# Deltares/xugrid

Hardware: AMD Instinct MI355X
Metric: target cells regridded/s (OverlapRegridder 1M->1M tri, weights + mean apply) (higher is better)
Workload: dtype f64; 1 GPU; BASELINE config 2: ~1M-triangle jittered-lattice Delaunay source -> ~1M-triangle target (seed 1, rotated 30 deg, scaled 0.7), OverlapRegridder area-weighted mean, K=1; target_faces=999660, candidate_pairs=6677422, nnz=4052965, parallelism=1 GPU

## Files before the change

xugrid_amd/csrc/xr_clip_tri.h:

```cpp
#pragma once

#include "xr_geom.h"

namespace xr {

static constexpr double TRI_AREA_OVERFLOW = -1.0;
static constexpr int TRI_MAXV = 6;
static constexpr int TRI_LUT = 64;

template <int MAXV>
__device__ __forceinline__ void poly_lut_init(uint2 *lut) {
    constexpr int N_LUT = 1 << MAXV;
    const int i = threadIdx.x;
    if (i >= N_LUT) return;
    uint32_t pos[8] = {MAXV, MAXV, MAXV, MAXV, MAXV, MAXV, MAXV, MAXV};
    if (i >= 8) {
        const int n = 31 - __clz(i);
        const uint32_t F = (uint32_t)i - (1u << n);
        int before = 0, n_t = 0;
        for (int j = 0; j < n; j++) {
            const bool fj = (F >> j) & 1u, fp = (F >> ((j + n - 1) % n)) & 1u;
            if (fj != fp) {
                if (n_t < 2) pos[5 + n_t] = (uint32_t)before;
                n_t++;
// ... 36 lines not shown
            const bool cross = live && (b_inside != a_inside);
            P2 pt{0.0, 0.0};
            bool have_pt = false;
            if (cross) {
                const double wx = r.x - a.x, wy = r.y - a.y;
                const double nw = N.x * wx + N.y * wy;
                const double nv = N.x * V.x + N.y * V.y;
                if (nv != 0) {
                    const double tt = nw / nv;
                    pt.x = a.x + tt * V.x;
                    pt.y = a.y + tt * V.y;
                    have_pt = true;
                }
            }
            const bool quirk = cross && !b_inside && !have_pt;
            if (cross && have_pt) {
                col[(n_output < MAXV ? n_output : MAXV) * STRIDE] = make_double2(pt.x, pt.y);
                n_output++;
            }
            b_inside = b_inside || quirk;
            if (live && b_inside) {
                col[(n_output < MAXV ? n_output : MAXV) * STRIDE] = make_double2(b.x, b.y);
                n_output++;
            }
            if (live) {
                a = b;
                a_inside = b_inside;
            }
        }
    }
    if (n_output > MAXV) {
        overflow = true;
        alive = false;
    } else if (n_output < 3) {
        alive = false;
    }
    n = n_output;
}

template <int MAXV, int NIN, int STRIDE, bool LAST = false>
__device__ __forceinline__ void poly_stage(int &n, P2 &r, const P2 s, bool &alive, bool &dirty, bool &overflow,
                                           double2 *col, const uint2 *lut) {
    const P2 U{s.x - r.x, s.y - r.y};
    const bool work = alive && !(U.x == 0 && U.y == 0);
    P2 v[MAXV];
#pragma unroll
    for (int j = 0; j < MAXV; j++) {
        if (j < NIN) {
            const double2 q = col[j * STRIDE];
            v[j] = P2{q.x, q.y};
        } else {
            v[j] = P2{0.0, 0.0};
        }
    }
    uint32_t F = 0;
#pragma unroll
    for (int j = 0; j < NIN; j++) F |= (U.x * (v[j].y - r.y) > U.y * (v[j].x - r.x)) ? (1u << j) : 0u;
    const uint32_t nmask = (1u << n) - 1u;
    F &= nmask;
    const uint32_t Tm = (F ^ ((F << 1) | (F >> ((n - 1) & 31)))) & nmask;
    const int n_tr = __popc(Tm);
    bool irregular = work && (dirty || n > NIN || (n_tr != 0 && n_tr != 2));
    const bool two = work && !irregular && n_tr == 2;
    if (two) {
        const int j1 = __ffs(Tm) - 1, j2 = 31 - __clz(Tm);
        const int p1 = j1 == 0 ? n - 1 : j1 - 1, p2 = j2 - 1;
        const double2 a1 = col[p1 * STRIDE], b1 = col[j1 * STRIDE], a2 = col[p2 * STRIDE], b2 = col[j2 * STRIDE];
        const uint2 e = lut[F + (1u << n)];
        const P2 N{-U.y, U.x};
        const P2 V1{b1.x - a1.x, b1.y - a1.y}, V2{b2.x - a2.x, b2.y - a2.y};
        const double nw1 = N.x * (r.x - a1.x) + N.y * (r.y - a1.y), nv1 = N.x * V1.x + N.y * V1.y;
        const double nw2 = N.x * (r.x - a2.x) + N.y * (r.y - a2.y), nv2 = N.x * V2.x + N.y * V2.y;
        const double tt1 = nw1 / nv1, tt2 = nw2 / nv2;
        const P2 pt1{a1.x + tt1 * V1.x, a1.y + tt1 * V1.y}, pt2{a2.x + tt2 * V2.x, a2.y + tt2 * V2.y};
        irregular = nv1 == 0 || nv2 == 0;
        if (!irregular) {
            if (!LAST && (pt1.x == a1.x || pt1.x == b1.x || pt2.x == a2.x || pt2.x == b2.x || pt1.x == pt2.x))
                dirty = p2_eq(pt1, a1) || p2_eq(pt1, b1) || p2_eq(pt2, a2) || p2_eq(pt2, b2) || p2_eq(pt1, pt2);
            *tri_slot<STRIDE>(col, e.x & 0xffu) = make_double2(v[0].x, v[0].y);
            *tri_slot<STRIDE>(col, (e.x >> 8) & 0xffu) = make_double2(v[1].x, v[1].y);
            *tri_slot<STRIDE>(col, (e.x >> 16) & 0xffu) = make_double2(v[2].x, v[2].y);
            if (NIN > 3) *tri_slot<STRIDE>(col, e.x >> 24) = make_double2(v[3].x, v[3].y);
            if (NIN > 4) *tri_slot<STRIDE>(col, e.y & 0xffu) = make_double2(v[4].x, v[4].y);
            if (NIN > 5) *tri_slot<STRIDE>(col, e.y >> 24) = make_double2(v[5].x, v[5].y);
            *tri_slot<STRIDE>(col, (e.y >> 8) & 0xffu) = make_double2(pt1.x, pt1.y);
            *tri_slot<STRIDE>(col, (e.y >> 16) & 0xffu) = make_double2(pt2.x, pt2.y);
            n = __popc(F) + 2;
        }
    } else if (work && !irregular && !(F & 1u)) {
        alive = false;
    }
    if (irregular) {
        if (n > NIN) {
#pragma unroll
            for (int j = NIN; j < MAXV; j++) {
                if (j < n) {
                    const double2 q = col[j * STRIDE];
                    v[j] = P2{q.x, q.y};
                }
            }
        }
        poly_stage_generic<MAXV, STRIDE>(v, n, r, U, alive, overflow, col);
        dirty = true;
    }
    if (work) r = s;
}

template <int MAXV, int N0, int STRIDE = 1>
__device__ __forceinline__ double poly_clip_area(const P2 (&tv)[N0], int n0, const P2 (&sv)[3], double2 *col, const uint2 *lut,
                                                 bool active) {
    int n = n0;
    bool alive = active, overflow = false;
    bool dirty = false;
#pragma unroll
    for (int j = 0; j < N0; j++)
        if (j < n0) dirty = dirty || p2_eq(tv[j], tv[j + 1 < n0 ? j + 1 : 0]);
    if (N0 > 3 && n0 > 3) dirty = dirty || p2_eq(tv[0], tv[2]) || p2_eq(tv[1], tv[3 < N0 ? 3 : 0]);
    if (active) {
#pragma unroll
        for (int j = 0; j < N0; j++)
            if (j < n0) col[j * STRIDE] = make_double2(tv[j].x, tv[j].y);
    }
    P2 r = sv[2];
    poly_stage<MAXV, N0, STRIDE>(n, r, sv[0], alive, dirty, overflow, col, lut);
    poly_stage<MAXV, N0 + 1, STRIDE>(n, r, sv[1], alive, dirty, overflow, col, lut);
    poly_stage<MAXV, N0 + 2, STRIDE, true>(n, r, sv[2], alive, dirty, overflow, col, lut);
    if (overflow) return TRI_AREA_OVERFLOW;
    double area = 0.0;
    if (alive) {
        const double2 q0 = col[0], q1 = col[STRIDE];
        const P2 a0{q0.x, q0.y};
        double ux = q1.x - a0.x, uy = q1.y - a0.y;
#pragma unroll
        for (int i = 2; i < MAXV; i++) {
            if (i < n) {
                const double2 q = col[i * STRIDE];
                const double vx = a0.x - q.x, vy = a0.y - q.y;
                area += fabs(ux * vy - uy * vx);
                ux = vx;
                uy = vy;
            }
        }
        area = 0.5 * area;
    }
    return area;
}

template <int STRIDE = 1>
__device__ __forceinline__ double tri_clip_area(const P2 (&tv)[3], const P2 (&sv)[3], double2 *col, const uint2 *lut,
                                                bool active) {
    return poly_clip_area<TRI_MAXV, 3, STRIDE>(tv, 3, sv, col, lut, active);
}

static constexpr int QUAD_MAXV = 7;
static constexpr int QUAD_LUT = 1 << QUAD_MAXV;

}
```

xugrid_amd/csrc/xr_overlap.hip:

```cpp
#include "xr_objects.h"
#include "xr_clip_tri.h"

namespace xr {

static constexpr int BIG_VISITS = 160;

__device__ __forceinline__ bool rec_hit(float4 b, float qx0, float qx1, float qy0, float qy1) {
    return box_gap(b, qx0, qx1, qy0, qy1) < 0.0f;
}

static constexpr int SLOTS = 16;
static constexpr int QCUR_STRIDE = 32;
static constexpr int TILE_RUN = 16;

__device__ __forceinline__ int64_t xcd_block(int64_t n_blocks, bool remap) {
    if (!remap) return blockIdx.x;
    const int64_t per_xcd = (n_blocks + 7) >> 3;
    return (int64_t)(blockIdx.x & 7) * per_xcd + (blockIdx.x >> 3);
}

static constexpr int WALK_PAD = 8;
static constexpr int BIGREC_MAX = 1024;
static constexpr int BIGREC_BLOCK = 64;

// ... 285 lines not shown
        if (slot_face && threadIdx.x == 0)
            slot_face[nb <= BIG_RANK_MAX ? sh_rankw[0] + sh_rankw[1] + sh_rankw[2] + sh_rankw[3] : bi] = t;
        if (threadIdx.x < np) sh_poly[threadIdx.x] = reinterpret_cast<const double2 *>(q_fxy)[face_vertex_base(q_off, t, q_m) + threadIdx.x];
        if (threadIdx.x == 0) sh_cursor = 0;
        __syncthreads();
        const double2 *poly = sh_poly;
        const double4 bb = reinterpret_cast<const double4 *>(q_bbox)[t];
        const float qx0 = f32_below(bb.x - g.x0), qx1 = f32_above(bb.y - g.x0);
        const float qy0 = f32_below(bb.z - g.y0), qy1 = f32_above(bb.w - g.y0);
        for (int pass = FUSED ? 0 : 1; pass < 2; pass++) {
        const bool STAGE = pass == 0;
        if (!STAGE) {
            if (FUSED) {
                __syncthreads();
                const int n = sh_cursor;
                __syncthreads();
                if (threadIdx.x == 0) {
                    const int base = atomicAdd(queue_cursor, n);
                    cand_count[t] = n;
                    cand_off[t] = base;
                    const bool fits = (int64_t)base + n <= capacity && base >= 0;
                    if (!fits) pending_list[atomicAdd(n_pending, 1)] = t;
                    sh_out0 = fits ? base : -1;
                    sh_cursor = 0;
                }
                __syncthreads();
                const int out = sh_out0;
                if (out < 0) break;
                if (n <= big_stage) {
                    for (int i = threadIdx.x; i < n; i += 256) {
                        cand_tgt[out + i] = t;
                        cand_src[out + i] = sh_stage[i];
                    }
                    break;
                }
            } else {
                if (threadIdx.x == 0) sh_out0 = cand_off[t];
                __syncthreads();
            }
            if (sh_out0 < 0) break;
        }
        const int out0 = STAGE ? 0 : sh_out0;
        for (int l = 0; l < g.n_levels; l++) {
            const double h = level_h(g, l), inv_h = level_inv_h(g, l);
            const double eps = 1e-6 * h;
            const int nx = g.nx[l], ny = g.ny[l], base = g.base[l];
            const int cy0 = cell_coord(bb.z - h, g.y0, inv_h, ny), cy1 = cell_coord(bb.w, g.y0, inv_h, ny);
            int batch_id = 0;
            for (int cyb = cy0; cyb <= cy1; cyb += 64, batch_id++) {
                if (((batch_id + l) & 3) != wv) continue;
                const int cy = cyb + lane;
                int r0 = 0, r1 = 0;
                float rx0 = qx0, rx1 = qx1;
                if (cy <= cy1) {
                    const double ya = g.y0 + (double)cy * h - eps, yb = g.y0 + (double)(cy + 2) * h + eps;
                    double xlo = INFINITY, xhi = -INFINITY;
                    double2 p = poly[np - 1];
                    for (int k = 0; k < np; k++) {
                        const double2 q = poly[k];
                        const double ylo = fmin(p.y, q.y), yhi = fmax(p.y, q.y);
                        if (yhi >= ya && ylo <= yb) {
                            double xa = p.x, xb = q.x;
                            if (yhi > ylo) {
                                const double inv = 1.0 / (q.y - p.y);
                                double t0 = (ya - p.y) * inv, t1 = (yb - p.y) * inv;
                                if (t0 > t1) { const double tmp = t0; t0 = t1; t1 = tmp; }
                                t0 = fmax(t0, 0.0);
                                t1 = fmin(t1, 1.0);
                                xa = p.x + t0 * (q.x - p.x);
                                xb = p.x + t1 * (q.x - p.x);
                            }
                            xlo = fmin(xlo, fmin(xa, xb));
                            xhi = fmax(xhi, fmax(xa, xb));
                        }
                        p = q;
                    }
                    if (xhi >= xlo) {
                        xlo = fmax(xlo - eps, bb.x);
                        xhi = fmin(xhi + eps, bb.y);
                        const int cx0 = cell_coord(xlo - h, g.x0, inv_h, nx), cx1 = cell_coord(xhi, g.x0, inv_h, nx);
                        r0 = cell_start[base + cy * nx + cx0];
                        r1 = cell_start[base + cy * nx + cx1 + 1];
                        rx0 = fmaxf(qx0, f32_below(xlo - g.x0));
                        rx1 = fminf(qx1, f32_above(xhi - g.x0));
                    }
                }
                const int len = r1 - r0;
                unsigned long long long_mask = __ballot(len > LONG_RUN);
                while (long_mask) {
                    const int src_lane = __ffsll((long long)long_mask) - 1;
                    long_mask &= long_mask - 1;
                    const int R0 = __shfl(r0, src_lane, 64), R1 = __shfl(r1, src_lane, 64);
                    const float X0 = __shfl(rx0, src_lane, 64), X1 = __shfl(rx1, src_lane, 64);
                    for (int rb = R0; rb < R1; rb += 64) {
                        const int r = rb + lane;
                        const bool hit = r < R1 && rec_hit(rbb[r], X0, X1, qy0, qy1);
                        const unsigned long long mask = __ballot(hit);
                        const int n = __popcll(mask);
                        if (n > 0) {
                            int slot0 = 0;
                            if (lane == 0) slot0 = atomicAdd(&sh_cursor, n);
                            slot0 = __shfl(slot0, 0, 64);
                            if (hit) {
                                const int slot = slot0 + __popcll(mask & lt_mask);
                                if (STAGE) {
                                    if (slot < big_stage) sh_stage[FUSED ? slot : 0] = r;
                                } else {
                                    cand_tgt[out0 + slot] = t;
                                    cand_src[out0 + slot] = r;
                                }
                            }
                        }
                    }
                }
                const int my_r1 = len > LONG_RUN ? r0 : r1;
                int cnt = 0;
                for (int r = r0; r < my_r1; r++) cnt += rec_hit(rbb[r], rx0, rx1, qy0, qy1) ? 1 : 0;
                const int excl = wave_excl_scan_i32(cnt, lane);
                const int batch = __shfl(excl + cnt, 63, 64);
                if (batch > 0) {
                    int slot0 = 0;
                    if (lane == 0) slot0 = atomicAdd(&sh_cursor, batch);
                    slot0 = __shfl(slot0, 0, 64);
                    int pos = slot0 + excl;
                    for (int r = r0; r < my_r1; r++) {
                        if (rec_hit(rbb[r], rx0, rx1, qy0, qy1)) {
                            if (STAGE) {
                                if (pos < big_stage) sh_stage[FUSED ? pos : 0] = r;
                            } else {
                                cand_tgt[out0 + pos] = t;
                                cand_src[out0 + pos] = r;
                            }
                            pos++;
                        }
                    }
                }
            }
        }
        }
    }
}

__device__ __forceinline__ bool pair_passes_box_and_sat(const double2 *__restrict__ a, int na, const double2 *__restrict__ b, int nb) {
    double ax0 = INFINITY, ax1 = -INFINITY, ay0 = INFINITY, ay1 = -INFINITY, bx0 = INFINITY, bx1 = -INFINITY, by0 = INFINITY, by1 = -INFINITY;
    for (int j = 0; j < na; j++) {
        const double2 q = a[j];
        ax0 = fmin(ax0, q.x), ax1 = fmax(ax1, q.x), ay0 = fmin(ay0, q.y), ay1 = fmax(ay1, q.y);
    }
    for (int j = 0; j < nb; j++) {
        const double2 q = b[j];
        bx0 = fmin(bx0, q.x), bx1 = fmax(bx1, q.x), by0 = fmin(by0, q.y), by1 = fmax(by1, q.y);
    }
    if (!(ax0 < bx1 && bx0 < ax1 && ay0 < by1 && by0 < ay1)) return false;
    for (int pass = 0; pass < 2; pass++) {
        const double2 *p = pass ? b : a;
        const int np = pass ? nb : na;
        for (int i = 0; i < np; i++) {
            const double2 v0 = p[i], v1 = p[i + 1 < np ? i + 1 : 0];
            const double nx = -(v1.y - v0.y), ny = v1.x - v0.x;
            if (nx == 0 && ny == 0) continue;
            double amin = INFINITY, amax = -INFINITY, bmin = INFINITY, bmax = -INFINITY;
            for (int j = 0; j < na; j++) {
                const double2 q = a[j];
                const double d = nx * q.x + ny * q.y;
                amin = d < amin ? d : amin;
                amax = d > amax ? d : amax;
            }
            for (int j = 0; j < nb; j++) {
                const double2 q = b[j];
                const double d = nx * q.x + ny * q.y;
                bmin = d < bmin ? d : bmin;
                bmax = d > bmax ? d : bmax;
            }
            if (amax < bmin || bmax < amin) return false;
        }
    }
    return true;
}
__device__ __forceinline__ double confirm_dust(double area, double dust, bool active, const double2 *__restrict__ a, int na,
                                               const double2 *__restrict__ b, int nb) {
    const bool suspicious = active && area > 0 && area <= dust;
    if (__any(suspicious)) {
        if (suspicious && !pair_passes_box_and_sat(a, na, b, nb)) area = 0.0;
    }
    return area;
}

__device__ __forceinline__ bool sh_inside(P2 p, P2 r, P2 U) { return U.x * (p.y - r.y) > U.y * (p.x - r.x); }

__device__ __forceinline__ bool sh_intersection(P2 a, P2 V, P2 r, P2 N, P2 &out) {
    const double wx = r.x - a.x, wy = r.y - a.y;
    const double nw = N.x * wx + N.y * wy;
    const double nv = N.x * V.x + N.y * V.y;
    if (nv != 0) {
        const double tt = nw / nv;
        out.x = a.x + tt * V.x;
        out.y = a.y + tt * V.y;
        return true;
    }
    return false;
}

static constexpr double AREA_OVERFLOW = -1.0;

template <int MAXV, int BLOCK>
__global__ void __launch_bounds__(BLOCK)
k_clip(const double *__restrict__ q_fxy, const uint8_t *__restrict__ q_len, const int32_t *__restrict__ q_off, int q_m,
       const int32_t *__restrict__ q_perm, const double *__restrict__ s_fxy, const uint8_t *__restrict__ s_len, const int32_t *__restrict__ s_off,
       int s_m, const int32_t *__restrict__ cand_tgt, const int32_t *__restrict__ cand_src, int64_t n_cand,
       double *__restrict__ cand_area, bool redo_only, const int32_t *__restrict__ rec_face,
       int32_t *__restrict__ cand_sid, int32_t *__restrict__ overflow_count, int32_t *__restrict__ nnz_row, double dust) {
    extern __shared__ __attribute__((aligned(16))) char smem[];
    double2 *sh = reinterpret_cast<double2 *>(smem);
    const int64_t c = (int64_t)blockIdx.x * BLOCK + threadIdx.x;
    const bool active = c < n_cand && !(redo_only && cand_area[c] != AREA_OVERFLOW);
    int t = -1;
    double area = 0.0;
    if (active) {
    t = cand_tgt[c];
    const int s = cand_src[c];
    cand_sid[c] = rec_face[s];
    const int nt = q_len[t], ns = s_len[s];
    double2 *out = sh + threadIdx.x;
    double2 *in = sh + MAXV * BLOCK + threadIdx.x;
    const double2 *tf = reinterpret_cast<const double2 *>(q_fxy) + face_vertex_base(q_off, t, q_m);
    const double *sf = s_fxy + 2 * face_vertex_base(s_off, s, s_m);
    for (int j = 0; j < nt; j++) out[j * BLOCK] = tf[j];
    int n_output = nt;
    bool overflow = false;
    P2 r = load_p2(sf, ns - 1);
    bool empty = false;
    for (int i = 0; i < ns; i++) {
        const P2 sv = load_p2(sf, i);
        const P2 U{sv.x - r.x, sv.y - r.y};
        if (U.x == 0 && U.y == 0) continue;
        const P2 N{-U.y, U.x};
        const int length = n_output;
        {
            double2 *tmp = in;
            in = out;
            out = tmp;
        }
        n_output = 0;
        const double2 a2 = in[(length - 1) * BLOCK];
        P2 a{a2.x, a2.y};
        bool a_inside = sh_inside(a, r, U);
        for (int j = 0; j < length; j++) {
            const double2 b2 = in[j * BLOCK];
            const P2 b{b2.x, b2.y};
            const P2 V{b.x - a.x, b.y - a.y};
            if (V.x == 0 && V.y == 0) continue;
            bool b_inside = sh_inside(b, r, U);
            if (b_inside) {
                if (!a_inside) {
                    P2 pt;
                    if (sh_intersection(a, V, r, N, pt)) {
                        if (n_output < MAXV) out[n_output * BLOCK] = make_double2(pt.x, pt.y);
                        else overflow = true;
                        n_output++;
                    }
                }
                if (n_output < MAXV) out[n_output * BLOCK] = b2;
                else overflow = true;
                n_output++;
            } else if (a_inside) {
                P2 pt;
                if (sh_intersection(a, V, r, N, pt)) {
                    if (n_output < MAXV) out[n_output * BLOCK] = make_double2(pt.x, pt.y);
                    else overflow = true;
                    n_output++;
                } else {
                    b_inside = true;
                    if (n_output < MAXV) out[n_output * BLOCK] = b2;
                    else overflow = true;
                    n_output++;
                }
            }
            a = b;
            a_inside = b_inside;
        }
        if (overflow) break;
        if (n_output < 3) {
            empty = true;
            break;
        }
        r = sv;
    }
    if (overflow) {
        area = AREA_OVERFLOW;
        atomicAdd(overflow_count, 1);
    } else if (!empty) {
        const double2 a2 = out[0];
        const double2 b2 = out[BLOCK];
        double ux = b2.x - a2.x, uy = b2.y - a2.y;
        for (int i = 2; i < n_output; i++) {
            const double2 c2 = out[i * BLOCK];
            const double vx = a2.x - c2.x, vy = a2.y - c2.y;
            area += fabs(ux * vy - uy * vx);
            ux = vx;
            uy = vy;
        }
        area = 0.5 * area;
    }
    if (area > 0 && area <= dust && !pair_passes_box_and_sat(tf, nt, reinterpret_cast<const double2 *>(sf), ns)) area = 0.0;
    cand_area[c] = area;
    }
    {
        const int lane = threadIdx.x & 63;
        const int t_prev = __shfl_up(t, 1, 64);
        const bool head = lane == 0 || t_prev != t;
        const unsigned long long heads = __ballot(head);
        const unsigned long long surv = __ballot(active && area > 0);
        if (head && t >= 0) {
            const unsigned long long above = lane == 63 ? 0ull : (heads >> (lane + 1));
            const int next = above ? lane + 1 + (__ffsll((long long)above) - 1) : 64;
            unsigned long long run = next == 64 ? ~0ull : ((1ull << next) - 1);
            run &= ~((1ull << lane) - 1);
            const int n = __popcll(surv & run);
            if (n > 0) atomicAdd(&nnz_row[t], n);
        }
    }
}

template <int MAXV, int BLOCK, bool TRI>
__device__ __forceinline__ double clip_small_pair(const double2 *__restrict__ tf, int nt, const double *__restrict__ sf, int ns,
                                                  double2 *out) {
    double area = 0.0;
    P2 in[MAXV];
    P2 last{0.0, 0.0};
// ... 998 lines not shown
```

xugrid_amd/csrc/xr_overlap_fused.h:

```cpp
#pragma once

namespace xr {

static constexpr int FB = 256;
static constexpr int FWAVES = FB / 64;

struct FusedCounters {
    int32_t n_apply_long;
    int32_t error;
    int32_t p_regular;
    int32_t rows_regular;
    int32_t p_big;
    int32_t pad0;
    int32_t max_row;
    int32_t pad2;
};

enum CtlWord : int {
    CTL_REG_CURSOR = 0,
    CTL_BIG_CURSOR = 1,
    CTL_N_BIG = 2,
    CTL_N_PENDING = 3,
    CTL_BIG_OVERFLOW = 4,
    CTL_COUNTERS = 8,
    CTL_LINE = 16,
    CTL_REGION_CURSOR = 32,
    CTL_WORDS = CTL_REGION_CURSOR + 8 * QCUR_STRIDE
};
#define XR_CTL_COUNTER(field) (xr::CTL_COUNTERS + (int)(offsetof(xr::FusedCounters, field) / sizeof(int32_t)))
static_assert(CTL_COUNTERS + sizeof(FusedCounters) / sizeof(int32_t) <= CTL_LINE && CTL_BIG_OVERFLOW < CTL_COUNTERS &&
                  CTL_LINE <= CTL_REGION_CURSOR && CTL_LINE + 8 <= 64,
              "the counters lie inside the line k_publish_all's one wave fetches, the region cursors behind it");
enum MailSlot : int {
    MAIL_REG_PAIRS = 0,
    MAIL_BIG_PAIRS = 1,
    MAIL_N_BIG = 2,
    MAIL_N_PENDING = 3,
    MAIL_BIG_OVERFLOW = 4,
    MAIL_ERROR = 5,
    MAIL_ROWS_REGULAR = 6,
    MAIL_N_APPLY_LONG = 7,
    MAIL_P_REGULAR = 8,
    MAIL_P_BIG = 9,
    MAIL_MAX_ROW = 10,
    MAIL_REGION_LEN = 11,
    MAIL_FUSED_SLOTS = MAIL_REGION_LEN + 8
};
static_assert(MAIL_BIG_OVERFLOW - MAIL_REG_PAIRS == CTL_BIG_OVERFLOW - CTL_REG_CURSOR && MAIL_FUSED_SLOTS <= MAIL_SEQ_SLOT,
              "the first control words map to the first mailbox slots one to one");

enum GenWord : int {
    GEN_CLIP_OVERFLOW = 0,
    GEN_N_PENDING = 1,
    GEN_N_LONG_ROWS = 1,
    GEN_N_BIG = 2,
    GEN_QUEUE_CURSOR = 3,
    GEN_WORDS = 4
};
enum GenMailSlot : int { GMAIL_PAIRS = 0, GMAIL_NNZ = 1, GMAIL_CLIP_OVERFLOW = 2, GMAIL_N_PENDING = 3 };

__device__ __forceinline__ int block_excl_scan(int v, int *sh_wave , int *total) {
    const int lane = threadIdx.x & 63, wave = threadIdx.x >> 6;
    int incl = v;
#pragma unroll
    for (int d = 1; d < 64; d <<= 1) {
        const int u = __shfl_up(incl, d, 64);
        if (lane >= d) incl += u;
    }
    __syncthreads();
    if (lane == 63) sh_wave[wave] = incl;
    __syncthreads();
    int woff = 0, tot = 0;
#pragma unroll
    for (int w = 0; w < FWAVES; w++) {
        if (w < wave) woff += sh_wave[w];
        tot += sh_wave[w];
    }
    *total = tot;
    return woff + incl - v;
}

template <int BLOCK, int COUNT, int KIND = 0>
__global__ void __launch_bounds__(BLOCK) __attribute__((amdgpu_waves_per_eu(KIND == 0 ? 5 : 4)))
k_clip_tri_queue(const double *__restrict__ q_fxy, const double *__restrict__ rec_fxy,
                 const int32_t *__restrict__ rec_face, const int32_t *cand_tgt,
                 const int32_t *cand_src, const int32_t *__restrict__ n_cand_dev, int64_t capacity,
                 double *__restrict__ cand_area, int32_t *__restrict__ cand_sid, int32_t *__restrict__ error_bits,
                 int32_t *__restrict__ nnz_row ,
                 const int32_t *__restrict__ skip_if ,
                 int32_t *__restrict__ blk_surv = nullptr ,
                 double dust = 0.0 ,
                 const uint8_t *__restrict__ q_len = nullptr, const uint8_t *__restrict__ s_len = nullptr, int q_m = 3, int s_m = 3) {
    extern __shared__ __attribute__((aligned(16))) char smem[];
    constexpr int CS = 1;
    constexpr int SMALL_MAXV = 8;
    double2 *col = reinterpret_cast<double2 *>(smem) + (KIND == 1 ? threadIdx.x : threadIdx.x * (TRI_MAXV + 1));
    __shared__ uint2 sh_lut[KIND == 1 ? 1 : TRI_LUT];
    if (skip_if) __builtin_amdgcn_s_setprio(3);
    if (skip_if && *skip_if > 0) return;
    if (KIND == 0) {
        tri_lut_init(sh_lut);
        __syncthreads();
    }
    const bool regions = capacity < 0;
    const int64_t region_cap = regions ? -capacity : 0;
    int64_t n_cand = 0, per_xcd;
    auto region_len = [&](int x) -> int64_t {
        const int64_t n = n_cand_dev[x * QCUR_STRIDE];
        return n < region_cap ? n : region_cap;
    };
    if (regions) {
        int64_t longest = 0;
#pragma unroll
        for (int x = 0; x < 8; x++) longest = region_len(x) > longest ? region_len(x) : longest;
        per_xcd = (longest + BLOCK - 1) / BLOCK;
    } else {
        n_cand = *n_cand_dev < capacity ? *n_cand_dev : capacity;
        per_xcd = ((n_cand + BLOCK - 1) / BLOCK + 7) >> 3;
    }
    const int64_t n_slots = per_xcd * 8;
    auto slot_first = [&](int64_t j, int64_t *end) -> int64_t {
        if (regions) {
            const int x = (int)(j & 7);
            *end = (int64_t)x * region_cap + region_len(x);
            return (int64_t)x * region_cap + (j >> 3) * BLOCK;
        }
        *end = n_cand;
        return ((j & 7) * per_xcd + (j >> 3)) * BLOCK;
    };
    const double2 *tfx = reinterpret_cast<const double2 *>(q_fxy);
    const double2 *sfx = reinterpret_cast<const double2 *>(rec_fxy);
    const int tid = threadIdx.x;
    int n_tq = 0, n_s = 0;
    auto load_idx = [&](int64_t slot, int &tq, int &s) {
        tq = 0;
        s = 0;
        if (slot < n_slots) {
            int64_t end;
            const int64_t c = slot_first(slot, &end) + tid;
            if (c < end) {
                tq = cand_tgt[c];
                s = cand_src[c];
            }
        }
    };
    const int64_t stride = gridDim.x;
    int64_t slot = blockIdx.x;
    load_idx(slot, n_tq, n_s);
    bool overflow = false;
    for (; slot < n_slots; slot += stride) {
        int64_t c_end;
        const int64_t c = slot_first(slot, &c_end) + tid;
        const bool active = c < c_end;
        int sid = 0;
        const int cur_tq = n_tq;
        double area = 0.0;
        if (KIND == 1) {
            const int cur_s = n_s;
            int nt = 0, ns = 0;
            if (active) {
                sid = rec_face[cur_s];
                nt = q_len[cur_tq];
                ns = s_len[cur_s];
            }
            load_idx(slot + stride, n_tq, n_s);
            if (active) {
                const double2 *tf = tfx + (int64_t)cur_tq * q_m;
                const double2 *sf = sfx + (int64_t)cur_s * s_m;
                area = clip_small_pair<SMALL_MAXV, BLOCK, false>(tf, nt, reinterpret_cast<const double *>(sf), ns, col);
                if (area > 0 && area <= dust && !pair_passes_box_and_sat(tf, nt, sf, ns)) area = 0.0;
            }
        } else {
            P2 tv[3] = {{0, 0}, {0, 0}, {0, 0}}, sv[3] = {{0, 0}, {0, 0}, {0, 0}};
            if (active) {
#pragma unroll
                for (int j = 0; j < 3; j++) {
                    const double2 a = tfx[(int64_t)n_tq * 3 + j], b2 = sfx[(int64_t)n_s * 3 + j];
                    tv[j] = P2{a.x, a.y};
                    sv[j] = P2{b2.x, b2.y};
                }
                sid = rec_face[n_s];
            }
            load_idx(slot + stride, n_tq, n_s);
            area = tri_clip_area<CS>(tv, sv, col, sh_lut, active);
            const bool suspicious = active && area > 0 && area <= dust;
            if (__any(suspicious)) {
                if (suspicious && !pair_passes_box_and_sat(tfx + (int64_t)cur_tq * 3, 3, sfx + (int64_t)cand_src[c] * 3, 3)) area = 0.0;
            }
        }
        const int tq_now = active ? cur_tq : -1;
        if (active) {
            overflow = overflow || area == TRI_AREA_OVERFLOW;
            cand_area[c] = area;
            cand_sid[c] = area > 0 ? sid : 0x7fffffff;
        }
        if (COUNT == 1) {
            const int lane = tid & 63;
            const int blk_now = active ? (cur_tq >> 8) : -1;
            const unsigned long long surv = __ballot(active && area > 0);
            const int blk_first = __builtin_amdgcn_readfirstlane(blk_now), blk_last = __shfl(blk_now, 63, 64);
            if (blk_first == blk_last) {
                if (lane == 0 && blk_first >= 0 && surv) atomicAdd(&blk_surv[blk_first], __popcll(surv));
            } else {
                const int blk_prev = __shfl_up(blk_now, 1, 64);
                const bool head = lane == 0 || blk_prev != blk_now;
                const unsigned long long heads = __ballot(head);
                if (head && blk_now >= 0) {
                    const unsigned long long above = lane == 63 ? 0ull : (heads >> (lane + 1));
                    const int next = above ? lane + 1 + (__ffsll((long long)above) - 1) : 64;
                    unsigned long long run = next == 64 ? ~0ull : ((1ull << next) - 1);
                    run &= ~((1ull << lane) - 1);
                    const int n = __popcll(surv & run);
                    if (n > 0) atomicAdd(&blk_surv[blk_now], n);
                }
            }
        }
        if (COUNT == 2) {
            const int lane = tid & 63;
            const int t_prev = __shfl_up(tq_now, 1, 64);
            const bool head = lane == 0 || t_prev != tq_now;
            const unsigned long long heads = __ballot(head);
            const unsigned long long surv = __ballot(active && area > 0);
            if (head && tq_now >= 0) {
                const unsigned long long above = lane == 63 ? 0ull : (heads >> (lane + 1));
                const int next = above ? lane + 1 + (__ffsll((long long)above) - 1) : 64;
                unsigned long long run = next == 64 ? ~0ull : ((1ull << next) - 1);
                run &= ~((1ull << lane) - 1);
                const int n = __popcll(surv & run);
                if (n > 0) atomicAdd(&nnz_row[tq_now], n);
            }
        }
    }
    if (overflow) atomicOr(error_bits, 1);
}

__global__ void __launch_bounds__(1024)
k_assemble_scan(const int32_t *__restrict__ blk_rows, const int32_t *__restrict__ blk_surv, int64_t n_blocks, int n_chain,
                bool remap, int32_t *__restrict__ base_rows, int32_t *__restrict__ base_nnz, FusedCounters *counters,
                int32_t *__restrict__ indptr) {
    __shared__ long long sh_w[16];
    __shared__ long long sh_carry;
    const int tid = threadIdx.x, lane = tid & 63, wave = tid >> 6;
    if (tid == 0) sh_carry = 0;
    __syncthreads();
    const int64_t per_xcd = (n_blocks + 7) >> 3;
    for (int b0 = 0; b0 < n_chain; b0 += 1024) {
        const int b = b0 + tid;
        long long v = 0;
        if (b < n_chain) {
            const int64_t lb = remap ? (int64_t)(b & 7) * per_xcd + (b >> 3) : b;
            if (lb < n_blocks) v = ((long long)blk_rows[lb] << 31) | (long long)blk_surv[lb];
        }
        long long incl = v;
#pragma unroll
        for (int d = 1; d < 64; d <<= 1) {
            const long long o = __shfl_up(incl, d, 64);
            if (lane >= d) incl += o;
        }
        if (lane == 63) sh_w[wave] = incl;
        __syncthreads();
        long long woff = 0, tot = 0;
        for (int w = 0; w < 16; w++) {
            if (w < wave) woff += sh_w[w];
            tot += sh_w[w];
        }
        const long long excl = sh_carry + woff + incl - v;
        if (b < n_chain) {
            base_nnz[b] = (int32_t)(excl & 0x7fffffffll);
            base_rows[b] = (int32_t)(excl >> 31);
        }
        __syncthreads();
        if (tid == 0) sh_carry += tot;
        __syncthreads();
    }
    if (tid == 0) {
        const long long entries = sh_carry & 0x7fffffffll, rows = sh_carry >> 31;
        counters->p_regular = (int32_t)entries;
        counters->rows_regular = (int32_t)rows;
        indptr[rows] = (int32_t)entries;
    }
}

__global__ void __launch_bounds__(FB, 2)
k_assemble(const double *__restrict__ q_bbox, const int32_t *__restrict__ q_perm, int64_t n_query,
           const int32_t *__restrict__ cand_tgt, const int32_t *__restrict__ cand_off,
           const int32_t *__restrict__ cand_count, const int2 *__restrict__ block_seg,
           const uint8_t *__restrict__ is_big, const double *__restrict__ cand_area,
           const int32_t *__restrict__ cand_sid, const double *__restrict__ src_area, bool relative, MortonParams tile,
           int32_t *__restrict__ tile_key, FusedCounters *__restrict__ counters,
           int32_t *__restrict__ indptr, int32_t *__restrict__ indices, double *__restrict__ data, int32_t *__restrict__ row_order,
           int32_t *__restrict__ apply_long_rows, int64_t csr_capacity, bool remap,
           const int32_t *__restrict__ base_rows = nullptr, const int32_t *__restrict__ base_nnz = nullptr,
           const int32_t *__restrict__ blk_rows = nullptr, const int32_t *__restrict__ blk_surv = nullptr) {
    __shared__ int32_t sh_stage[SLOTS * FB];
    __shared__ int32_t sh_nnz[FB];
    __shared__ uint16_t sh_lo[FB];
    __shared__ uint16_t sh_rowoff[FB];
    __shared__ uint8_t sh_cnt[FB];
    __shared__ int32_t sh_wave[FWAVES];
    __shared__ long long sh_base;
    const int tid = threadIdx.x;
    const int64_t n_blocks = (n_query + FB - 1) / FB;
    const int64_t lb = xcd_block(n_blocks, remap);
    const bool valid_block = lb < n_blocks;
    sh_nnz[tid] = 0;
    const int64_t t0 = lb * FB;
    const int64_t t = t0 + tid;
    const bool in_range = valid_block && t < n_query;
    const int2 seg = valid_block ? block_seg[lb] : make_int2(0, 0);
    const int total = seg.y;
    bool regular = false;
    int my_cnt = 0;
    if (in_range) {
        regular = !is_big[t];
        my_cnt = regular ? cand_count[t] : 0;
        sh_lo[tid] = (uint16_t)(regular ? cand_off[t] - seg.x : 0);
    } else {
        sh_lo[tid] = 0;
    }
    sh_cnt[tid] = (uint8_t)my_cnt;
    __syncthreads();
    for (int i0 = tid; i0 < total; i0 += 4 * FB) {
        int s[4], row[4];
#pragma unroll
        for (int u = 0; u < 4; u++) {
            const int i = i0 + u * FB;
            const int64_t c = (int64_t)seg.x + (i < total ? i : total - 1);
            s[u] = cand_sid[c];
            row[u] = cand_tgt[c] - (int)t0;
        }
#pragma unroll
        for (int u = 0; u < 4; u++) {
            const int i = i0 + u * FB;
            if (i < total) {
                sh_stage[i] = s[u];
                if (s[u] != 0x7fffffff) atomicAdd(&sh_nnz[row[u]], 1);
            }
        }
    }
    __syncthreads();
    const int my_nnz = regular ? sh_nnz[tid] : 0;
    int block_nnz = 0, block_rows = 0;
    const int rowoff = block_excl_scan(my_nnz, sh_wave, &block_nnz);
    const int rowidx = block_excl_scan(regular ? 1 : 0, sh_wave, &block_rows);
    sh_rowoff[tid] = (uint16_t)rowoff;
    const int b = (int)blockIdx.x, n_chain = (int)gridDim.x;
    if (blk_surv) {
        const int64_t per_xcd = (n_blocks + 7) >> 3;
        long long acc = 0;
        for (int hb = tid; hb < b; hb += FB) {
            const int64_t plb = remap ? (int64_t)(hb & 7) * per_xcd + (hb >> 3) : hb;
            if (plb < n_blocks) acc += ((long long)blk_rows[plb] << 31) | (long long)blk_surv[plb];
        }
#pragma unroll
        for (int d = 32; d > 0; d >>= 1) acc += __shfl_xor(acc, d, 64);
        __shared__ long long sh_part[FWAVES];
        if ((tid & 63) == 0) sh_part[tid >> 6] = acc;
        __syncthreads();
        if (tid == 0) {
            long long tot = 0;
#pragma unroll
            for (int w = 0; w < FWAVES; w++) tot += sh_part[w];
            sh_base = tot;
        }
    } else {
        if (tid == 0) sh_base = ((long long)base_rows[b] << 31) | (long long)base_nnz[b];
    }
    __syncthreads();
    const long long base = sh_base & 0x7fffffffll, row_base = sh_base >> 31;
// ... 131 lines not shown
```

Baseline: 2.073 billion target cells/s.

## Prefilter separated triangle pairs with SAT and compact survivors via per-wave ring

For the triangle KIND=0/COUNT=1 path, each candidate pair is first tested with a cheap separating-axis check on the target's edges. Separated pairs are marked dead right away. Survivors are compacted into a per-wavefront shared-memory ring, and the expensive clip runs only on full waves of 64 live pairs. This cuts the divergence and wasted lanes spent clipping pairs with no overlap, at the cost of extra loads, shared-memory traffic and a reload of vertex data for the popped entries. The SAT loop and the block-survivor counting are also factored into helpers.

```diff
diff --git a/xugrid_amd/csrc/xr_clip_tri.h b/xugrid_amd/csrc/xr_clip_tri.h
--- a/xugrid_amd/csrc/xr_clip_tri.h
+++ b/xugrid_amd/csrc/xr_clip_tri.h
@@ -212,6 +212,35 @@
     return poly_clip_area<TRI_MAXV, 3, STRIDE>(tv, 3, sv, col, lut, active);
 }
 
+template <class VP, class VA, class VB>
+__host__ __device__ __forceinline__ bool sat_axes_separate(const VP *p, int np, const VA *a, int na, const VB *b, int nb) {
+    for (int i = 0; i < np; i++) {
+        const VP v0 = p[i], v1 = p[i + 1 < np ? i + 1 : 0];
+        const double nx = -(v1.y - v0.y), ny = v1.x - v0.x;
+        if (nx == 0 && ny == 0) continue;
+        double amin = INFINITY, amax = -INFINITY, bmin = INFINITY, bmax = -INFINITY;
+        for (int j = 0; j < na; j++) {
+            const VA q = a[j];
+            const double d = nx * q.x + ny * q.y;
+            amin = d < amin ? d : amin;
+            amax = d > amax ? d : amax;
+        }
+        for (int j = 0; j < nb; j++) {
+            const VB q = b[j];
+            const double d = nx * q.x + ny * q.y;
+            bmin = d < bmin ? d : bmin;
+            bmax = d > bmax ? d : bmax;
+        }
+        if (amax < bmin || bmax < amin) return true;
+    }
+    return false;
+}
+
+__host__ __device__ __forceinline__ bool tri_pair_separated(const P2 (&tv)[3], const P2 (&sv)[3]) {
+    const bool point = sv[0].x == sv[1].x && sv[0].y == sv[1].y && sv[1].x == sv[2].x && sv[1].y == sv[2].y;
+    return !point && sat_axes_separate(tv, 3, tv, 3, sv, 3);
+}
+
 static constexpr int QUAD_MAXV = 7;
 static constexpr int QUAD_LUT = 1 << QUAD_MAXV;
 
diff --git a/xugrid_amd/csrc/xr_overlap.hip b/xugrid_amd/csrc/xr_overlap.hip
--- a/xugrid_amd/csrc/xr_overlap.hip
+++ b/xugrid_amd/csrc/xr_overlap.hip
@@ -461,29 +461,8 @@
         bx0 = fmin(bx0, q.x), bx1 = fmax(bx1, q.x), by0 = fmin(by0, q.y), by1 = fmax(by1, q.y);
     }
     if (!(ax0 < bx1 && bx0 < ax1 && ay0 < by1 && by0 < ay1)) return false;
-    for (int pass = 0; pass < 2; pass++) {
-        const double2 *p = pass ? b : a;
-        const int np = pass ? nb : na;
-        for (int i = 0; i < np; i++) {
-            const double2 v0 = p[i], v1 = p[i + 1 < np ? i + 1 : 0];
-            const double nx = -(v1.y - v0.y), ny = v1.x - v0.x;
-            if (nx == 0 && ny == 0) continue;
-            double amin = INFINITY, amax = -INFINITY, bmin = INFINITY, bmax = -INFINITY;
-            for (int j = 0; j < na; j++) {
-                const double2 q = a[j];
-                const double d = nx * q.x + ny * q.y;
-                amin = d < amin ? d : amin;
-                amax = d > amax ? d : amax;
-            }
-            for (int j = 0; j < nb; j++) {
-                const double2 q = b[j];
-                const double d = nx * q.x + ny * q.y;
-                bmin = d < bmin ? d : bmin;
-                bmax = d > bmax ? d : bmax;
-            }
-            if (amax < bmin || bmax < amin) return false;
-        }
-    }
+    for (int pass = 0; pass < 2; pass++)
+        if (sat_axes_separate(pass ? b : a, pass ? nb : na, a, na, b, nb)) return false;
     return true;
 }
 __device__ __forceinline__ double confirm_dust(double area, double dust, bool active, const double2 *__restrict__ a, int na,
diff --git a/xugrid_amd/csrc/xr_overlap_fused.h b/xugrid_amd/csrc/xr_overlap_fused.h
--- a/xugrid_amd/csrc/xr_overlap_fused.h
+++ b/xugrid_amd/csrc/xr_overlap_fused.h
@@ -80,6 +80,26 @@
     return woff + incl - v;
 }
 
+__device__ __forceinline__ void add_block_survivors(int32_t *__restrict__ blk_surv, int blk_now, bool alive, int lane) {
+    const unsigned long long surv = __ballot(alive);
+    const int blk_first = __builtin_amdgcn_readfirstlane(blk_now), blk_last = __shfl(blk_now, 63, 64);
+    if (blk_first == blk_last) {
+        if (lane == 0 && blk_first >= 0 && surv) atomicAdd(&blk_surv[blk_first], __popcll(surv));
+    } else {
+        const int blk_prev = __shfl_up(blk_now, 1, 64);
+        const bool head = lane == 0 || blk_prev != blk_now;
+        const unsigned long long heads = __ballot(head);
+        if (head && blk_now >= 0) {
+            const unsigned long long above = lane == 63 ? 0ull : (heads >> (lane + 1));
+            const int next = above ? lane + 1 + (__ffsll((long long)above) - 1) : 64;
+            unsigned long long run = next == 64 ? ~0ull : ((1ull << next) - 1);
+            run &= ~((1ull << lane) - 1);
+            const int n = __popcll(surv & run);
+            if (n > 0) atomicAdd(&blk_surv[blk_now], n);
+        }
+    }
+}
+
 template <int BLOCK, int COUNT, int KIND = 0>
 __global__ void __launch_bounds__(BLOCK) __attribute__((amdgpu_waves_per_eu(KIND == 0 ? 5 : 4)))
 k_clip_tri_queue(const double *__restrict__ q_fxy, const double *__restrict__ rec_fxy,
@@ -148,6 +168,79 @@
     int64_t slot = blockIdx.x;
     load_idx(slot, n_tq, n_s);
     bool overflow = false;
+    if constexpr (KIND == 0 && COUNT == 1) {
+        constexpr int RING = 128;
+        __shared__ uint32_t sh_ring[BLOCK / 64][RING];
+        uint32_t *const ring = sh_ring[tid >> 6];
+        const bool prefilter = dust > 0;
+        int head = 0, fill = 0;
+        auto clip_popped = [&](bool act) {
+            const uint32_t *const entry = &ring[(head + (tid & 63)) & (RING - 1)];
+            P2 tv[3] = {{0, 0}, {0, 0}, {0, 0}}, sv[3] = {{0, 0}, {0, 0}, {0, 0}};
+            int tq = 0, sid = 0;
+            if (act) {
+                const int64_t c = *entry;
+                tq = cand_tgt[c];
+                const int s = cand_src[c];
+#pragma unroll
+                for (int j = 0; j < 3; j++) {
+                    const double2 a = tfx[(int64_t)tq * 3 + j], b2 = sfx[(int64_t)s * 3 + j];
+                    tv[j] = P2{a.x, a.y};
+                    sv[j] = P2{b2.x, b2.y};
+                }
+                sid = rec_face[s];
+            }
+            double area = tri_clip_area<CS>(tv, sv, col, sh_lut, act);
+            const int64_t c = *entry;
+            const bool suspicious = act && area > 0 && area <= dust;
+            if (__any(suspicious)) {
+                if (suspicious && !pair_passes_box_and_sat(tfx + (int64_t)tq * 3, 3, sfx + (int64_t)cand_src[c] * 3, 3)) area = 0.0;
+            }
+            if (act) {
+                overflow = overflow || area == TRI_AREA_OVERFLOW;
+                cand_area[c] = area;
+                cand_sid[c] = area > 0 ? sid : 0x7fffffff;
+            }
+            add_block_survivors(blk_surv, act ? (tq >> 8) : -1, act && area > 0, tid & 63);
+        };
+        for (;; slot += stride) {
+            const bool more = slot < n_slots;
+            if (more) {
+                int64_t c_end;
+                const int64_t c = slot_first(slot, &c_end) + tid;
+                const bool active = c < c_end;
+                bool keep = active;
+                {
+                    P2 tv[3] = {{0, 0}, {0, 0}, {0, 0}}, sv[3] = {{0, 0}, {0, 0}, {0, 0}};
+                    if (active) {
+#pragma unroll
+                        for (int j = 0; j < 3; j++) {
+                            const double2 a = tfx[(int64_t)n_tq * 3 + j], b2 = sfx[(int64_t)n_s * 3 + j];
+                            tv[j] = P2{a.x, a.y};
+                            sv[j] = P2{b2.x, b2.y};
+                        }
+                    }
+                    load_idx(slot + stride, n_tq, n_s);
+                    if (prefilter && tri_pair_separated(tv, sv)) keep = false;
+                }
+                if (active && !keep) cand_sid[c] = 0x7fffffff;
+                const unsigned long long kept = __ballot(keep);
+                const int rank = __builtin_amdgcn_mbcnt_hi((uint32_t)(kept >> 32), __builtin_amdgcn_mbcnt_lo((uint32_t)kept, 0u));
+                if (keep) ring[(head + fill + rank) & (RING - 1)] = (uint32_t)c;
+                fill += __popcll(kept);
+                __builtin_amdgcn_fence(__ATOMIC_ACQ_REL, "wavefront");
+            }
+            const int n_pop = fill >= 64 ? 64 : (more ? 0 : fill);
+            if (n_pop > 0) {
+                clip_popped((tid & 63) < n_pop);
+                head = (head + n_pop) & (RING - 1);
+                fill -= n_pop;
+            }
+            if (!more) break;
+        }
+        if (overflow) atomicOr(error_bits, 1);
+        return;
+    }
     for (; slot < n_slots; slot += stride) {
         int64_t c_end;
         const int64_t c = slot_first(slot, &c_end) + tid;
@@ -194,27 +287,7 @@
             cand_area[c] = area;
             cand_sid[c] = area > 0 ? sid : 0x7fffffff;
         }
-        if (COUNT == 1) {
-            const int lane = tid & 63;
-            const int blk_now = active ? (cur_tq >> 8) : -1;
-            const unsigned long long surv = __ballot(active && area > 0);
-            const int blk_first = __builtin_amdgcn_readfirstlane(blk_now), blk_last = __shfl(blk_now, 63, 64);
-            if (blk_first == blk_last) {
-                if (lane == 0 && blk_first >= 0 && surv) atomicAdd(&blk_surv[blk_first], __popcll(surv));
-            } else {
-                const int blk_prev = __shfl_up(blk_now, 1, 64);
-                const bool head = lane == 0 || blk_prev != blk_now;
-                const unsigned long long heads = __ballot(head);
-                if (head && blk_now >= 0) {
-                    const unsigned long long above = lane == 63 ? 0ull : (heads >> (lane + 1));
-                    const int next = above ? lane + 1 + (__ffsll((long long)above) - 1) : 64;
-                    unsigned long long run = next == 64 ? ~0ull : ((1ull << next) - 1);
-                    run &= ~((1ull << lane) - 1);
-                    const int n = __popcll(surv & run);
-                    if (n > 0) atomicAdd(&blk_surv[blk_now], n);
-                }
-            }
-        }
+        if (COUNT == 1) add_block_survivors(blk_surv, active ? (cur_tq >> 8) : -1, active && area > 0, tid & 63);
         if (COUNT == 2) {
             const int lane = tid & 63;
             const int t_prev = __shfl_up(tq_now, 1, 64);
```

Result: slower. 2.024 billion target cells/s (-2.4%).
